# sdiehl/sonic

Hardware: AMD Instinct MI355X
Metric: prove() proofs/sec (higher is better)
Workload: dtype u32 limbs (Fq 12x32, Fr 8x32 Montgomery); 1 GPU; prove(): rndCircuit n=2^18, Q=2, SRS d=2^21 (d=8n >= 7n, Protocol.hs:54); n=262144, Q=2, d=2097152, process_group=none (plain single-process run), legs=headline only (the other legs: --full)

## Files before the change

### sonic_amd/csrc/field.hpp

```cpp
#pragma once
#include <stdint.h>
#include "constants.hpp"

#if defined(__HIP_DEVICE_COMPILE__) && !defined(SONIC_NO_ASM_MUL)
#define SONIC_FQ_LAZY 1
#else
#define SONIC_FQ_LAZY 0
#endif

#if defined(__HIPCC__)
#define HD __host__ __device__ __forceinline__
#define HD_NOINLINE __host__ __device__ __attribute__((noinline))
#else
#define HD inline __attribute__((always_inline))
#define HD_NOINLINE inline
#endif

namespace sonic {

struct FqParams {
  static constexpr int N = FQ_LIMBS;
  static constexpr uint32_t INV = FQ_INV;
  static constexpr bool LAZY = SONIC_FQ_LAZY != 0;
  static HD constexpr uint32_t p(int i) { constexpr uint32_t v[N] = FQ_P; return v[i]; }
// ... 177 lines not shown
    for (int j = 1; j < M; j++) {
      c += (u128)m * Pm[j] + t[j];
      t[j - 1] = (uint64_t)c;
      c >>= 64;
    }
    c += t[M];
    t[M - 1] = (uint64_t)c;
    t[M] = t[M + 1] + (uint64_t)(c >> 64);
  }
  Fp<P> r;
  for (int i = 0; i < M; i++) { r.l[2 * i] = (uint32_t)t[i]; r.l[2 * i + 1] = (uint32_t)(t[i] >> 32); }
  fp_reduce_once(r);
  return r;
}
#endif

}
#include "mont_asm.hpp"
namespace sonic {

template <class P>
HD Fp<P> fp_mul(const Fp<P>& a, const Fp<P>& b) {
#if defined(__HIP_DEVICE_COMPILE__) && !defined(SONIC_NO_ASM_MUL)
  if constexpr (P::N == FQ_LIMBS) return sonic_mont_mul_fq_call(a, b);
  else return sonic_mont_mul_fr_call(a, b);
#elif defined(__HIP_DEVICE_COMPILE__)
  return fp_mul_generic(a, b);
#else
  return fp_mul_host64(a, b);
#endif
}

template <class P>
HD Fp<P> fp_add(const Fp<P>& a, const Fp<P>& b) {
#if defined(__HIP_DEVICE_COMPILE__) && !defined(SONIC_NO_ASM_MUL)
  if constexpr (P::N == FQ_LIMBS) return sonic_fq_add_asm<P>(a, b);
  else return sonic_fr_add_asm<P>(a, b);
#else
  return fp_add_generic(a, b);
#endif
}
template <class P>
HD Fp<P> fp_sub(const Fp<P>& a, const Fp<P>& b) {
#if defined(__HIP_DEVICE_COMPILE__) && !defined(SONIC_NO_ASM_MUL)
  if constexpr (P::N == FQ_LIMBS) return sonic_fq_sub_asm<P>(a, b);
  else return sonic_fr_sub_asm<P>(a, b);
#else
  return fp_sub_generic(a, b);
#endif
}
template <class P>
HD Fp<P> fp_dbl(const Fp<P>& a) { return fp_add(a, a); }

template <class P>
HD Fp<P> fp_sqr(const Fp<P>& a) {
#if defined(__HIP_DEVICE_COMPILE__) && !defined(SONIC_NO_ASM_MUL)
  if constexpr (P::N == FQ_LIMBS) return sonic_mont_sqr_fq_call(a);
  else return fp_mul(a, a);
#else
  return fp_mul(a, a);
#endif
}

template <class P>
HD Fp<P> fp_to_mont(const Fp<P>& a) { return fp_mul(a, Fp<P>::r2()); }

template <class P>
HD Fp<P> fp_canonical(const Fp<P>& a) {
  Fp<P> r = a;
  if constexpr (P::LAZY) fp_reduce_once(r);
  return r;
}

template <class P>
HD bool Fp<P>::operator==(const Fp<P>& o) const {
  if constexpr (P::LAZY) return fp_sub(*this, o).is_zero();
  uint32_t t = 0;
  for (int i = 0; i < N; i++) t |= l[i] ^ o.l[i];
  return t == 0;
}

template <class P>
HD Fp<P> fp_from_mont(const Fp<P>& a) {
  Fp<P> o = Fp<P>::zero();
  o.l[0] = 1;
  return fp_canonical(fp_mul(a, o));
}

template <class P>
HD Fp<P> fp_pow_u64(const Fp<P>& a, uint64_t e) {
  Fp<P> acc = Fp<P>::one();
  bool started = false;
  for (int i = 63; i >= 0; i--) {
    if (started) acc = fp_sqr(acc);
    if ((e >> i) & 1) { acc = fp_mul(acc, a); started = true; }
  }
  return acc;
}

#if !defined(__HIP_DEVICE_COMPILE__)
template <class P>
inline Fp<P> fp_inv_euclid(const Fp<P>& a) {
  constexpr int N = P::N;
  if (a.is_zero()) return Fp<P>::zero();
  uint32_t u[N], v[N], x1[N], x2[N], pm[N];
  for (int i = 0; i < N; i++) { u[i] = a.l[i]; v[i] = pm[i] = P::p(i); x1[i] = 0; x2[i] = 0; }
// ... 84 lines not shown
```

### sonic_amd/csrc/g1.hpp

```cpp
#pragma once
#include "field.hpp"

namespace sonic {

struct G1Affine {
  Fq x, y;
  HD bool is_inf() const { return x.is_zero_strict() && y.is_zero_strict(); }
  static HD G1Affine inf() { G1Affine p; p.x = Fq::zero(); p.y = Fq::zero(); return p; }
};

#ifndef SONIC_SRS_POINT_BYTES
#define SONIC_SRS_POINT_BYTES 128
#endif
struct PointArray {
  const char* p;
  uint32_t stride;
  HD const G1Affine& operator[](size_t i) const { return *reinterpret_cast<const G1Affine*>(p + i * (size_t)stride); }
  HD PointArray operator+(long i) const { return PointArray{p + i * (long)stride, stride}; }
  static HD PointArray packed(const G1Affine* a) { return PointArray{reinterpret_cast<const char*>(a), (uint32_t)sizeof(G1Affine)}; }
};
struct PointArrayMut {
  char* p;
  uint32_t stride;
  HD G1Affine& operator[](size_t i) const { return *reinterpret_cast<G1Affine*>(p + i * (size_t)stride); }
  HD PointArrayMut operator+(long i) const { return PointArrayMut{p + i * (long)stride, stride}; }
  HD operator PointArray() const { return PointArray{p, stride}; }
};

struct G1XYZZ {
  Fq x, y, zz, zzz;
  HD bool is_inf() const { return zz.is_zero_strict(); }
  static HD G1XYZZ inf() {
    G1XYZZ p; p.x = Fq::zero(); p.y = Fq::zero(); p.zz = Fq::zero(); p.zzz = Fq::zero(); return p;
  }
  static HD G1XYZZ from_affine(const G1Affine& a) {
    G1XYZZ p;
    if (a.is_inf()) return inf();
    p.x = a.x; p.y = a.y; p.zz = Fq::one(); p.zzz = Fq::one();
    return p;
  }
};

HD G1Affine g1_neg(const G1Affine& p) { G1Affine r; r.x = p.x; r.y = fp_neg(p.y); return r; }
HD G1XYZZ g1_neg(const G1XYZZ& p) { G1XYZZ r = p; r.y = fp_neg(p.y); return r; }

HD G1XYZZ g1_dbl_affine(const G1Affine& p) {
  if (p.is_inf() || p.y.is_zero()) return G1XYZZ::inf();
  G1XYZZ r;
  Fq U = fp_dbl(p.y);
  Fq V = fp_sqr(U);
  Fq W = fp_mul(U, V);
  Fq S = fp_mul(p.x, V);
  Fq X2 = fp_sqr(p.x);
  Fq M = fp_add(fp_dbl(X2), X2);
  r.x = fp_sub(fp_sqr(M), fp_dbl(S));
  r.y = fp_sub(fp_mul(M, fp_sub(S, r.x)), fp_mul(W, p.y));
  r.zz = V;
  r.zzz = W;
  return r;
}

HD G1XYZZ g1_dbl(const G1XYZZ& p) {
  if (p.is_inf() || p.y.is_zero()) return G1XYZZ::inf();
  G1XYZZ r;
  Fq U = fp_dbl(p.y);
  Fq V = fp_sqr(U);
  Fq W = fp_mul(U, V);
  Fq S = fp_mul(p.x, V);
  Fq X2 = fp_sqr(p.x);
  Fq M = fp_add(fp_dbl(X2), X2);
  r.x = fp_sub(fp_sqr(M), fp_dbl(S));
  r.y = fp_sub(fp_mul(M, fp_sub(S, r.x)), fp_mul(W, p.y));
  r.zz = fp_mul(V, p.zz);
  r.zzz = fp_mul(W, p.zzz);
  return r;
}

HD G1XYZZ g1_add_mixed(const G1XYZZ& acc, const G1Affine& q) {
  if (q.is_inf()) return acc;
  if (acc.is_inf()) return G1XYZZ::from_affine(q);
  Fq U2 = fp_mul(q.x, acc.zz);
  Fq S2 = fp_mul(q.y, acc.zzz);
  Fq Pp = fp_sub(U2, acc.x);
  Fq R = fp_sub(S2, acc.y);
  if (Pp.is_zero()) {
    if (R.is_zero()) return g1_dbl_affine(q);
    return G1XYZZ::inf();
  }
  G1XYZZ r;
  Fq PP = fp_sqr(Pp);
  Fq PPP = fp_mul(Pp, PP);
  Fq Qv = fp_mul(acc.x, PP);
  r.x = fp_sub(fp_sub(fp_sqr(R), PPP), fp_dbl(Qv));
  r.y = fp_sub(fp_mul(R, fp_sub(Qv, r.x)), fp_mul(acc.y, PPP));
  r.zz = fp_mul(acc.zz, PP);
  r.zzz = fp_mul(acc.zzz, PPP);
  return r;
}

HD bool g1_in_subgroup_walk(const G1Affine& p) {
  constexpr uint32_t rl[8] = FR_P;
  G1XYZZ acc = G1XYZZ::from_affine(p);
#pragma unroll 1
  for (int b = 253; b >= 0; b--) {
    acc = g1_dbl(acc);
    uint32_t wd = 0;
#pragma unroll
    for (int k = 0; k < 8; k++) if (k == (b >> 5)) wd = rl[k];
    if ((wd >> (b & 31)) & 1u) acc = g1_add_mixed(acc, p);
  }
  return acc.is_inf();
}

HD Fq g1_endo_beta() {
  constexpr uint32_t b[12] = ENDO_BETA_MONT;
  Fq beta;
  for (int i = 0; i < 12; i++) beta.l[i] = b[i];
  return beta;
}

HD bool g1_in_subgroup(const G1Affine& p) {
  G1XYZZ acc = G1XYZZ::from_affine(p);
#pragma unroll 1
  for (int k = 0; k < 2; k++) {
    uint64_t w = k == 0 ? ENDO_Z2_HI << 1 : ENDO_Z2_LO;
    int left = k == 0 ? 63 : 64;
#pragma unroll 1
    while (left > 0) {
      const int run = w ? __builtin_clzll(w) + 1 : left;
#pragma unroll 1
      for (int i = 0; i < run; i++) acc = g1_dbl(acc);
      if (w) acc = g1_add_mixed(acc, p);
      w = run < 64 ? w << run : 0;
      left -= run;
    }
  }
  acc = g1_add_mixed(acc, g1_neg(p));
  if (acc.is_inf()) return false;
  return fp_mul(fp_mul(p.x, g1_endo_beta()), acc.zz) == acc.x && fp_mul(p.y, acc.zzz) == acc.y;
}

HD G1XYZZ g1_add_mixed_walk(G1XYZZ acc, const G1Affine& q, uint32_t negy = 0) {
#if SONIC_FQ_LAZY && !defined(SONIC_NO_FUSED_MADD)
  const uint32_t special = (acc.is_inf() || q.is_inf()) ? 1u : 0u;
  if (sonic_g1_madd_asm(acc, q.x, q.y, special, negy)) {
    G1Affine t = q;
    if (negy) t.y = fp_neg(t.y);
    acc = g1_add_mixed(acc, t);
  }
  return acc;
#else
  G1Affine t = q;
  if (negy) t.y = fp_neg(t.y);
  return g1_add_mixed(acc, t);
#endif
}

HD G1XYZZ g1_add_affine_walk(const G1Affine& first, const G1Affine& q, bool first_only) {
#if SONIC_FQ_LAZY && !defined(SONIC_NO_FUSED_MADD)
  G1XYZZ acc;
  acc.x = first.x; acc.y = first.y; acc.zz = Fq::one(); acc.zzz = Fq::one();
  const uint32_t special = (first_only || first.is_inf() || q.is_inf()) ? 1u : 0u;
  if (sonic_g1_aadd_asm(acc, q.x, q.y, special)) {
    acc = G1XYZZ::from_affine(first);
    if (!first_only) acc = g1_add_mixed(acc, q);
  }
  return acc;
#else
  G1XYZZ acc = G1XYZZ::from_affine(first);
  return first_only ? acc : g1_add_mixed(acc, q);
#endif
}

HD G1XYZZ g1_add(const G1XYZZ& p, const G1XYZZ& q) {
  if (q.is_inf()) return p;
  if (p.is_inf()) return q;
  Fq U1 = fp_mul(p.x, q.zz);
  Fq U2 = fp_mul(q.x, p.zz);
  Fq S1 = fp_mul(p.y, q.zzz);
  Fq S2 = fp_mul(q.y, p.zzz);
  Fq Pp = fp_sub(U2, U1);
  Fq R = fp_sub(S2, S1);
  if (Pp.is_zero()) {
    if (R.is_zero()) return g1_dbl(p);
    return G1XYZZ::inf();
  }
  G1XYZZ r;
  Fq PP = fp_sqr(Pp);
  Fq PPP = fp_mul(Pp, PP);
  Fq Qv = fp_mul(U1, PP);
  r.x = fp_sub(fp_sub(fp_sqr(R), PPP), fp_dbl(Qv));
  r.y = fp_sub(fp_mul(R, fp_sub(Qv, r.x)), fp_mul(S1, PPP));
  r.zz = fp_mul(fp_mul(p.zz, q.zz), PP);
  r.zzz = fp_mul(fp_mul(p.zzz, q.zzz), PPP);
  return r;
}

HD G1Affine g1_to_affine(const G1XYZZ& p) {
  if (p.is_inf()) return G1Affine::inf();
  Fq i = fp_inv(fp_mul(p.zz, p.zzz));
  G1Affine r;
  r.x = fp_mul(p.x, fp_mul(i, p.zzz));
  r.y = fp_mul(p.y, fp_mul(i, p.zz));
  return r;
}

HD G1XYZZ g1_mul_small(const G1XYZZ& p, uint32_t k) {
  G1XYZZ acc = G1XYZZ::inf();
  bool started = false;
  for (int i = 31; i >= 0; i--) {
    if (started) acc = g1_dbl(acc);
    if ((k >> i) & 1) { acc = g1_add(acc, p); started = true; }
  }
  return acc;
}

}
```

### sonic_amd/csrc/mont_asm.hpp

```cpp
#pragma once
#if defined(__HIP_DEVICE_COMPILE__)
namespace sonic {
extern "C" __device__ __attribute__((noinline, used)) void sonic_mont_mul_fq_holder() {
  asm volatile(
      ".pushsection .text.sonic_mont_mul_fq,\"ax\",@progbits\n\t"
      ".p2align 8\n\t"
      ".type sonic_mont_mul_fq,@function\n\t"
      "sonic_mont_mul_fq:\n\t"
      "s_mov_b32 s36, 0xffffaaab\n\t"
      "s_mov_b32 s37, 0xb9feffff\n\t"
      "s_mov_b32 s38, 0xb153ffff\n\t"
      "s_mov_b32 s39, 0x1eabfffe\n\t"
      "s_mov_b32 s40, 0xf6b0f624\n\t"
      "s_mov_b32 s41, 0x6730d2a0\n\t"
      "s_mov_b32 s42, 0xf38512bf\n\t"
      "s_mov_b32 s43, 0x64774b84\n\t"
      "s_mov_b32 s44, 0x434bacd7\n\t"
      "s_mov_b32 s45, 0x4b1ba7b6\n\t"
      "s_mov_b32 s46, 0x397fe69a\n\t"
      "s_mov_b32 s47, 0x1a0111ea\n\t"
      "s_mov_b32 s48, 0xfffcfffd\n\t"
      "v_mad_u64_u32 v[50:51], s[54:55], v0, v12, 0\n\t"
      "v_mad_u64_u32 v[52:53], s[54:55], v1, v12, 0\n\t"
      "v_mad_u64_u32 v[54:55], s[54:55], v2, v12, 0\n\t"
// ... 3727 lines not shown
      "v_mad_u64_u32 v[66:67], s[54:55], v107, v98, v[40:41]\n\t"
      "v_addc_co_u32_e64 v34, s[52:53], v60, v59, s[52:53]\n\t"
      "v_mad_u64_u32 v[56:57], s[54:55], v74, s39, v[30:31]\n\t"
      "v_addc_co_u32_e32 v46, vcc, v72, v71, vcc\n\t"
      "v_mad_u64_u32 v[68:69], s[54:55], v108, v98, v[42:43]\n\t"
      "v_addc_co_u32_e64 v36, s[52:53], v62, v61, s[52:53]\n\t"
      "v_mad_u64_u32 v[58:59], s[54:55], v74, s40, v[32:33]\n\t"
      "v_add_co_u32_e64 v24, s[50:51], v52, v51\n\t"
      "v_addc_co_u32_e32 v48, vcc, v48, v73, vcc\n\t"
      "v_mad_u64_u32 v[70:71], s[54:55], v109, v98, v[44:45]\n\t"
      "v_addc_co_u32_e64 v38, s[52:53], v64, v63, s[52:53]\n\t"
      "v_mad_u64_u32 v[60:61], s[54:55], v74, s41, v[34:35]\n\t"
      "v_addc_co_u32_e64 v26, s[50:51], v54, v53, s[50:51]\n\t"
      "v_mad_u64_u32 v[72:73], s[54:55], v110, v98, v[46:47]\n\t"
      "v_addc_co_u32_e64 v40, s[52:53], v66, v65, s[52:53]\n\t"
      "v_mad_u64_u32 v[62:63], s[54:55], v74, s42, v[36:37]\n\t"
      "v_addc_co_u32_e64 v28, s[50:51], v56, v55, s[50:51]\n\t"
      "v_addc_co_u32_e64 v42, s[52:53], v68, v67, s[52:53]\n\t"
      "v_mad_u64_u32 v[64:65], s[54:55], v74, s43, v[38:39]\n\t"
      "v_addc_co_u32_e64 v30, s[50:51], v58, v57, s[50:51]\n\t"
      "v_addc_co_u32_e64 v44, s[52:53], v70, v69, s[52:53]\n\t"
      "v_mad_u64_u32 v[66:67], s[54:55], v74, s44, v[40:41]\n\t"
      "v_addc_co_u32_e64 v32, s[50:51], v60, v59, s[50:51]\n\t"
      "v_addc_co_u32_e64 v46, s[52:53], v72, v71, s[52:53]\n\t"
      "v_mad_u64_u32 v[68:69], s[54:55], v74, s45, v[42:43]\n\t"
      "v_addc_co_u32_e64 v34, s[50:51], v62, v61, s[50:51]\n\t"
      "v_addc_co_u32_e64 v48, s[52:53], v48, v73, s[52:53]\n\t"
      "v_mad_u64_u32 v[70:71], s[54:55], v74, s46, v[44:45]\n\t"
      "v_addc_co_u32_e64 v36, s[50:51], v64, v63, s[50:51]\n\t"
      "v_mad_u64_u32 v[72:73], s[54:55], v74, s47, v[46:47]\n\t"
      "s_nop 0\n\t"
      "v_addc_co_u32_e64 v38, s[50:51], v66, v65, s[50:51]\n\t"
      "s_nop 0\n\t"
      "s_nop 0\n\t"
      "v_addc_co_u32_e64 v40, s[50:51], v68, v67, s[50:51]\n\t"
      "s_nop 0\n\t"
      "s_nop 0\n\t"
      "v_addc_co_u32_e64 v42, s[50:51], v70, v69, s[50:51]\n\t"
      "s_nop 0\n\t"
      "s_nop 0\n\t"
      "v_addc_co_u32_e64 v44, s[50:51], v72, v71, s[50:51]\n\t"
      "s_nop 0\n\t"
      "s_nop 0\n\t"
      "v_addc_co_u32_e64 v46, s[50:51], v48, v73, s[50:51]\n\t"
      "s_nop 0\n\t"
      "s_nop 0\n\t"
      "v_addc_co_u32_e64 v48, s[50:51], 0, 0, s[50:51]\n\t"
      "s_setpc_b64 s[30:31]\n\t"
      ".size sonic_mont_mul2_fq_core, .-sonic_mont_mul2_fq_core\n\t"
      ".popsection\n\t"
  );
}

template <class XYZZ, class F> __device__ __forceinline__ bool sonic_g1_madd_asm(XYZZ& acc, const F& qx, const F& qy, uint32_t special, uint32_t negy) {
  uint32_t exc;
  asm volatile(
      "s_mov_b32 s36, 0xffffaaab\n\t"
      "s_mov_b32 s37, 0xb9feffff\n\t"
      "s_mov_b32 s38, 0xb153ffff\n\t"
      "s_mov_b32 s39, 0x1eabfffe\n\t"
      "s_mov_b32 s40, 0xf6b0f624\n\t"
      "s_mov_b32 s41, 0x6730d2a0\n\t"
      "s_mov_b32 s42, 0xf38512bf\n\t"
      "s_mov_b32 s43, 0x64774b84\n\t"
      "s_mov_b32 s44, 0x434bacd7\n\t"
      "s_mov_b32 s45, 0x4b1ba7b6\n\t"
      "s_mov_b32 s46, 0x397fe69a\n\t"
      "s_mov_b32 s47, 0x1a0111ea\n\t"
      "s_mov_b32 s48, 0xfffcfffd\n\t"
      "v_mov_b32_e32 v25, 0\n\t"
      "v_mov_b32_e32 v27, 0\n\t"
      "v_mov_b32_e32 v29, 0\n\t"
      "v_mov_b32_e32 v31, 0\n\t"
      "v_mov_b32_e32 v33, 0\n\t"
      "v_mov_b32_e32 v35, 0\n\t"
      "v_mov_b32_e32 v37, 0\n\t"
      "v_mov_b32_e32 v39, 0\n\t"
      "v_mov_b32_e32 v41, 0\n\t"
      "v_mov_b32_e32 v43, 0\n\t"
      "v_mov_b32_e32 v45, 0\n\t"
      "v_mov_b32_e32 v47, 0\n\t"
      "v_mov_b32_e32 v49, 0\n\t"
      "v_mov_b32_e32 v48, 0\n\t"
      "s_mov_b64 s[60:61], exec\n\t"
      "v_cmp_ne_u32_e64 s[66:67], 0, %74\n\t"
      "v_sub_co_u32_e32 v50, vcc, 0xffff5556, %61\n\t"
      "v_mov_b32_e32 v63, 0x73fdffff\n\t"
      "v_mov_b32_e32 v64, 0x62a7ffff\n\t"
      "v_subb_co_u32_e32 v51, vcc, v63, %62, vcc\n\t"
      "v_mov_b32_e32 v65, 0x3d57fffd\n\t"
      "v_mov_b32_e32 v66, 0xed61ec48\n\t"
      "v_subb_co_u32_e32 v52, vcc, v64, %63, vcc\n\t"
      "v_mov_b32_e32 v67, 0xce61a541\n\t"
      "v_mov_b32_e32 v68, 0xe70a257e\n\t"
      "v_subb_co_u32_e32 v53, vcc, v65, %64, vcc\n\t"
      "v_mov_b32_e32 v69, 0xc8ee9709\n\t"
      "v_mov_b32_e32 v70, 0x869759ae\n\t"
      "v_subb_co_u32_e32 v54, vcc, v66, %65, vcc\n\t"
      "v_mov_b32_e32 v71, 0x96374f6c\n\t"
      "v_mov_b32_e32 v72, 0x72ffcd34\n\t"
      "v_subb_co_u32_e32 v55, vcc, v67, %66, vcc\n\t"
      "v_mov_b32_e32 v73, 0x340223d4\n\t"
      "v_mov_b32_e32 v12, %36\n\t"
      "v_subb_co_u32_e32 v56, vcc, v68, %67, vcc\n\t"
      "v_mov_b32_e32 v13, %37\n\t"
      "v_mov_b32_e32 v14, %38\n\t"
// ... 9185 lines not shown
```

### sonic_amd/csrc/msm.hip

```cpp
#include <string.h>
#include <stdexcept>
#include "internal.hpp"
#include "g1_quad.hpp"
#include "endo.hpp"

namespace sonic {

#ifndef SONIC_PART_LOW_BITS
#define SONIC_PART_LOW_BITS 8
#endif
constexpr int PART_LOW_BITS = SONIC_PART_LOW_BITS;
#ifndef SONIC_PART_TILE
#define SONIC_PART_TILE 1024
#endif
constexpr int PART_TILE = SONIC_PART_TILE;
constexpr uint32_t PASS1_GRID = 1024;
constexpr uint32_t PART_SORT_GRID = 2048;
#ifndef SONIC_PART_SORT_THREADS
#define SONIC_PART_SORT_THREADS 1024
#endif
constexpr int PART_SORT_THREADS = SONIC_PART_SORT_THREADS;
#ifndef SONIC_PART_SCATTER_THREADS
#define SONIC_PART_SCATTER_THREADS 512
#endif
constexpr int PART_SCATTER_THREADS = SONIC_PART_SCATTER_THREADS;
static_assert(PART_TILE % PART_SCATTER_THREADS == 0 && PART_SCATTER_THREADS >= 256, "a tile is a whole number of rounds of the workgroup");
static_assert(PART_LOW_BITS >= 8 && PART_LOW_BITS <= 10, "k_part_sort scans 256 x {1, 2, 4} counters");

static int g_window_override = 0;
int msm_window_override() { return g_window_override; }
void msm_set_window_override(int c) { g_window_override = c; }

#ifndef SONIC_HEAVY_THREADS
#define SONIC_HEAVY_THREADS 512
#endif
#ifndef SONIC_HEAVY_GRID
#define SONIC_HEAVY_GRID 256
#endif
static constexpr int HEAVY_THREADS = SONIC_HEAVY_THREADS;
static constexpr int HEAVY_GRID = SONIC_HEAVY_GRID;
static constexpr uint32_t HEAVY_MIN_STRETCH = 4 * HEAVY_THREADS;

struct HeavyMeta { uint32_t pad, n_heavy; uint32_t class_hist[256]; uint32_t class_cursor[256]; };
struct HeavyRec { uint32_t bucket, cnt, base, npart; };

static void plan_finish(MsmPlan& p, long n) {
  p.NB = 1 << (p.c - 1);
  p.K = p.NB < 8 ? p.NB : 8;
  p.nseg = p.NB / p.K;
  long mean = n * (long)(p.W / p.Wb) / p.NB;
  long t = 8 * mean;
  if (t < 256) t = 256;
  p.heavy_threshold = (uint32_t)t;
}

void msm_plan_set_segment(MsmPlan& p, int K) {
  if (K > p.NB) K = p.NB;
  if (K < 1) K = 1;
  while (K & (K - 1)) K &= K - 1;
  p.K = K;
  p.nseg = p.NB / K;
}

MsmPlan msm_plan(long n, bool fold) {
  MsmPlan p;
  p.fold = fold;
  int lg = 0;
  while ((1L << (lg + 1)) <= n) lg++;
  int c = lg - 4;
  if (c < 4) c = 4;
  if (c > 16) c = 16;
  if (g_window_override >= 4 && g_window_override <= 16) c = g_window_override;
  p.c = c;
  p.W = ((fold ? 255 : 256) + c - 1) / c;
// ... 220 lines not shown
    for (int k = 0; scans && k < per; k++) {
      const int t = threadIdx.x * per + k;
      if (t < P) { cur[t] = ex; delta[t] = base[row0 + (size_t)t * nblk] - ex; ex += hist[row0 + (size_t)t * nblk]; }
    }
    if (threadIdx.x == 0) total_sh = tot;
    __syncthreads();
    for (int k = 0; k < PART_TILE / T; k++) {
      const long i = (long)blk * PART_TILE + k * T + threadIdx.x;
      DigitStream ds;
      ds.init(scal, i, i < n, mont, fold);
      for (int w = 0; w < W; w++) {
        uint32_t sign;
        const uint32_t d = ds.next(keystride ? c : msm_even_width(W, w, batch.bits), sign);
        const uint32_t key = (uint32_t)w * keystride + d - 1;
        const uint32_t pr = key >> PART_LOW_BITS;
        const uint32_t pos = lds_take(cur, d != 0, pr);
        if (d) {
          const uint32_t lo = key & ((1u << PART_LOW_BITS) - 1), hi = (uint32_t)i | (keystride ? 0u : (uint32_t)w << 26) | (sign << 31);
          recs[pos] = make_uint2(lo, hi);
          pid[pos] = (uint16_t)pr;
        }
      }
    }
    __syncthreads();
    const uint32_t total = total_sh;
    for (uint32_t i = threadIdx.x; i < total; i += T) part[delta[pid[i]] + i] = recs[i];
    __syncthreads();
  }
}

__global__ __launch_bounds__(PART_SORT_THREADS) void k_part_sort(const MsmBatchDev batch, const uint2* __restrict__ part,
                                                   const uint32_t* __restrict__ base, const uint32_t* __restrict__ total, size_t hn, int P,
                                                   uint32_t jobstride, uint32_t* __restrict__ off, uint32_t* __restrict__ entries, uint32_t* __restrict__ class_hist,
                                                   uint32_t stage_cap) {
  extern __shared__ uint32_t stage[];
  __shared__ uint32_t cnt[1 << PART_LOW_BITS];
  __shared__ uint32_t sc4[256];
  __shared__ uint32_t chist[256];
  const uint32_t M = (uint32_t)batch.k * jobstride;
  const uint32_t nparts = (uint32_t)batch.k * (uint32_t)P;
  constexpr uint32_t T = PART_SORT_THREADS;
  if (threadIdx.x < 256) chist[threadIdx.x] = 0;
  for (uint32_t pi = blockIdx.x; pi < nparts; pi += gridDim.x) {
  const int job = pi / P, t = pi % P;
  const uint32_t nblk = batch.tile0[job + 1] - batch.tile0[job];
  const size_t idx = (size_t)P * batch.tile0[job] + (size_t)t * nblk, idx_next = idx + nblk;
  const uint32_t beg = idx < hn ? base[idx] : *total;
  const uint32_t end = idx_next < hn ? base[idx_next] : *total;
  const bool last_block = pi == nparts - 1;
  for (int t = threadIdx.x; t < (1 << PART_LOW_BITS); t += T) cnt[t] = 0;
  __syncthreads();
  const uint32_t span = end - beg, trips = (span + T - 1) / T;
  constexpr int B = 8;
  for (uint32_t k0 = 0; k0 < trips; k0 += B) {
    uint32_t lo[B];
#pragma unroll
    for (int j = 0; j < B; j++) { const uint32_t e = beg + (k0 + j) * T + threadIdx.x; lo[j] = e < end ? part[e].x : 0xffffffffu; }
#pragma unroll
    for (int j = 0; j < B; j++) if (k0 + j < trips) lds_take(cnt, lo[j] != 0xffffffffu, lo[j] & ((1u << PART_LOW_BITS) - 1));
  }
  __syncthreads();
  constexpr int CPT = (1 << PART_LOW_BITS) / 256;
  const bool scans = threadIdx.x < 256;
  uint32_t v[CPT], ssum = 0;
  for (int k = 0; k < CPT; k++) { v[k] = scans ? cnt[threadIdx.x * CPT + k] : 0u; ssum += v[k]; }
  uint32_t ex = block_exclusive_scan_256(ssum, sc4, nullptr);
  for (int k = 0; scans && k < CPT; k++) {
    const uint32_t local = (uint32_t)t * (1u << PART_LOW_BITS) + threadIdx.x * CPT + k;
    cnt[threadIdx.x * CPT + k] = ex;
    if (local < jobstride) { off[(uint32_t)job * jobstride + local] = beg + ex; atomicAdd(&chist[size_class(v[k])], 1u); }
    ex += v[k];
  }
  if (last_block && threadIdx.x == 0) off[M] = *total;
  __syncthreads();
  for (uint32_t k0 = 0; k0 < trips; k0 += B) {
    uint32_t lo[B], pay[B];
#pragma unroll
    for (int j = 0; j < B; j++) {
      const uint32_t e = beg + (k0 + j) * T + threadIdx.x;
      const bool live = e < end;
      const uint2 rec = live ? part[e] : make_uint2(0xffffffffu, 0u);
      lo[j] = rec.x;
      pay[j] = rec.y;
    }
#pragma unroll
    for (int j = 0; j < B; j++) {
      if (k0 + j >= trips) continue;
      const bool live = lo[j] != 0xffffffffu;
      const uint32_t pos = lds_take(cnt, live, lo[j] & ((1u << PART_LOW_BITS) - 1));
      if (live) { if (span <= stage_cap) stage[pos] = pay[j]; else entries[beg + pos] = pay[j]; }
    }
  }
  __syncthreads();
  if (span <= stage_cap) {
    for (uint32_t i = threadIdx.x; i < span; i += T) entries[beg + i] = stage[i];
    __syncthreads();
  }
  }
  const uint32_t c = threadIdx.x < 256 ? chist[threadIdx.x] : 0u;
  if (c) atomicAdd(&class_hist[threadIdx.x], c);
}

__device__ __forceinline__ uint32_t block_exclusive_scan_256(uint32_t v, uint32_t* sh, uint32_t* total) {
  const int t = threadIdx.x;
  const bool in = t < 256;
  if (in) sh[t] = v;
  __syncthreads();
  for (int o = 1; o < 256; o <<= 1) {
    uint32_t x = in && t >= o ? sh[t - o] : 0;
    __syncthreads();
    if (in) sh[t] += x;
    __syncthreads();
  }
  uint32_t incl = in ? sh[t] : 0u;
  if (total) *total = sh[255];
  __syncthreads();
  return incl - v;
}
__global__ __launch_bounds__(256) void k_scan_tile_sums(const uint32_t* in, size_t m, uint32_t* tile_sums) {
  __shared__ uint32_t sh[256];
  size_t base = (size_t)blockIdx.x * 2048 + threadIdx.x * 8;
  uint32_t s = 0;
  for (int k = 0; k < 8; k++) if (base + k < m) s += in[base + k];
  uint32_t tot;
  block_exclusive_scan_256(s, sh, &tot);
  if (threadIdx.x == 0) tile_sums[blockIdx.x] = tot;
}
__global__ __launch_bounds__(256) void k_scan_top(uint32_t* tile_sums, int ntiles, uint32_t* total_out) {
  __shared__ uint32_t sh[256];
  __shared__ uint32_t carry_sh;
  if (threadIdx.x == 0) carry_sh = 0;
  __syncthreads();
  for (int base = 0; base < ntiles; base += 256) {
    int idx = base + threadIdx.x;
    uint32_t v = idx < ntiles ? tile_sums[idx] : 0, tot;
    uint32_t ex = block_exclusive_scan_256(v, sh, &tot);
    uint32_t carry = carry_sh;
    if (idx < ntiles) tile_sums[idx] = ex + carry;
    __syncthreads();
    if (threadIdx.x == 0) carry_sh = carry + tot;
    __syncthreads();
  }
  if (threadIdx.x == 0) *total_out = carry_sh;
}
// ... 237 lines not shown
    }
    reinterpret_cast<Fq*>(&sh[q])[cr] = acc;
    __syncthreads();
    for (int sp = 8; sp >= 1; sp >>= 1) {
      if (q < sp && (uint32_t)(q + sp) < r.npart) {
        Fq* pa = reinterpret_cast<Fq*>(&sh[q]) + cr;
        *pa = g1q_add(*pa, reinterpret_cast<const Fq*>(&sh[q + sp])[cr], cr);
      }
      __syncthreads();
    }
    if (threadIdx.x < 4) reinterpret_cast<Fq*>(&buckets[r.bucket])[threadIdx.x] = reinterpret_cast<const Fq*>(&sh[0])[threadIdx.x];
    __syncthreads();
  }
}

#ifndef SONIC_SEGMENTS_LDS_TOT
#define SONIC_SEGMENTS_LDS_TOT 1
#endif
struct LdsPoint {
  uint32_t* base;
  __device__ __forceinline__ void store(const G1XYZZ& p) const {
    const uint32_t* w = reinterpret_cast<const uint32_t*>(&p);
#pragma unroll
    for (int k = 0; k < 48; k++) base[k * 256] = w[k];
  }
  __device__ __forceinline__ G1XYZZ load() const {
    G1XYZZ p;
    uint32_t* w = reinterpret_cast<uint32_t*>(&p);
#pragma unroll
    for (int k = 0; k < 48; k++) w[k] = base[k * 256];
    return p;
  }
  __device__ __forceinline__ Fq coord(int i) const {
    Fq f;
#pragma unroll
    for (int k = 0; k < 12; k++) f.l[k] = base[(12 * i + k) * 256];
    return f;
  }
  __device__ __forceinline__ void set_coord(int i, const Fq& f) const {
#pragma unroll
    for (int k = 0; k < 12; k++) base[(12 * i + k) * 256] = f.l[k];
  }
  __device__ __forceinline__ void add(const G1XYZZ& q) const {
    if (q.is_inf()) return;
    const Fq pzz = coord(2);
    if (pzz.is_zero_strict()) { store(q); return; }
    const Fq U1 = fp_mul(coord(0), q.zz);
    const Fq U2 = fp_mul(q.x, pzz);
    const Fq S1 = fp_mul(coord(1), q.zzz);
    const Fq S2 = fp_mul(q.y, coord(3));
    const Fq Pp = fp_sub(U2, U1);
    const Fq R = fp_sub(S2, S1);
    if (Pp.is_zero()) {
      store(R.is_zero() ? g1_dbl(load()) : G1XYZZ::inf());
      return;
    }
    const Fq PP = fp_sqr(Pp);
    const Fq PPP = fp_mul(Pp, PP);
    const Fq Qv = fp_mul(U1, PP);
    const Fq x = fp_sub(fp_sub(fp_sqr(R), PPP), fp_dbl(Qv));
    set_coord(0, x);
    set_coord(1, fp_sub(fp_mul(R, fp_sub(Qv, x)), fp_mul(S1, PPP)));
    set_coord(2, fp_mul(fp_mul(coord(2), q.zz), PP));
    set_coord(3, fp_mul(fp_mul(coord(3), q.zzz), PPP));
  }
};
template <bool RUNS>
__global__ __launch_bounds__(256, SONIC_SEGMENTS_LDS_TOT ? 2 : 1) void k_bucket_segments(const G1XYZZ* __restrict__ buckets, int W, int NB, int K, int nseg,
                                                        G1XYZZ* __restrict__ segres, G1XYZZ* __restrict__ runs) {
#if SONIC_SEGMENTS_LDS_TOT
  __shared__ uint32_t tot_sh[48 * 256];
  const LdsPoint tl{tot_sh + threadIdx.x};
#endif
  int t = blockIdx.x * blockDim.x + threadIdx.x;
  if (t >= W * nseg) return;
  const int w = t / nseg, sg = t % nseg;
  const G1XYZZ* B = buckets + (size_t)w * NB + (size_t)sg * K;
  G1XYZZ run = G1XYZZ::inf();
#if SONIC_SEGMENTS_LDS_TOT
  tl.store(G1XYZZ::inf());
  for (int j = K - 1; j >= 0; j--) {
    run = g1_add(run, B[j]);
    tl.add(run);
  }
#else
  G1XYZZ tot = G1XYZZ::inf();
  for (int j = K - 1; j >= 0; j--) {
    run = g1_add(run, B[j]);
    tot = g1_add(tot, run);
  }
#endif
  if (RUNS) {
    runs[t] = run;
#if SONIC_SEGMENTS_LDS_TOT
    segres[t] = tl.load();
#else
    segres[t] = tot;
#endif
    return;
  }
  const int k0 = sg * K;
  G1XYZZ acc = G1XYZZ::inf();
  bool have_multiple = false;
  if (nseg % 64 == 0) {
    const uint32_t hi = __builtin_amdgcn_readfirstlane((uint32_t)sg >> 6), lo = (uint32_t)sg & 63u;
    for (int i = 31 - __clz((int)(hi | 1u)); i >= 0; i--) {
      acc = g1_dbl(acc);
      if ((hi >> i) & 1u) acc = g1_add(acc, run);
    }
    for (int i = 5; i >= 0; i--) {
      acc = g1_dbl(acc);
      if ((lo >> i) & 1u) acc = g1_add(acc, run);
    }
    for (int s = K; s > 1; s >>= 1) acc = g1_dbl(acc);
    have_multiple = true;
  } else if (k0) {
    acc = g1_mul_small(run, (uint32_t)k0);
    have_multiple = true;
  }
#if SONIC_SEGMENTS_LDS_TOT
  G1XYZZ tot = tl.load();
#endif
  if (have_multiple) tot = g1_add(tot, acc);
  segres[t] = tot;
}

__global__ __launch_bounds__(256, 2) void k_window_sum(const G1XYZZ* __restrict__ segres, int W, int c, int nseg, int runs_L, int K, const MsmBatchDev batch) {
  __shared__ G1XYZZ sh[256];
  const int w = blockIdx.x % W;
  MsmSlot* slot = batch.slot[blockIdx.x / W];
  segres += (size_t)(blockIdx.x - w) * nseg;
  G1XYZZ acc = G1XYZZ::inf();
  for (int s = threadIdx.x; s < nseg; s += 256) acc = g1_add(acc, segres[(size_t)w * nseg + s]);
  sh[threadIdx.x] = acc;
  __syncthreads();
  for (int s = 128; s >= 1; s >>= 1) {
    if ((int)threadIdx.x < s) sh[threadIdx.x] = g1_add(sh[threadIdx.x], sh[threadIdx.x + s]);
    __syncthreads();
  }
  if (threadIdx.x == 0) {
    G1XYZZ r = sh[0];
    r.x = fp_canonical(r.x); r.y = fp_canonical(r.y); r.zz = fp_canonical(r.zz); r.zzz = fp_canonical(r.zzz);
    if (runs_L > 0) { slot->win[runs_L] = r; slot->W = runs_L; slot->c = 1; slot->pad0 = K; slot->pad1 = 3; return; }
    slot->win[w] = r;
    if (w == 0) { slot->W = W; slot->c = c; slot->pad0 = 0; slot->pad1 = 0; }
  }
}

__global__ __launch_bounds__(256, 2) void k_group_sum(const G1XYZZ* __restrict__ in, long n_in, int group, G1XYZZ* __restrict__ out) {
  __shared__ G1XYZZ sh[256];
  const long base = (long)blockIdx.x * group;
  G1XYZZ acc = G1XYZZ::inf();
  for (long s = threadIdx.x; s < group && base + s < n_in; s += 256) acc = g1_add(acc, in[base + s]);
  sh[threadIdx.x] = acc;
  __syncthreads();
  for (int s = 128; s >= 1; s >>= 1) {
    if ((int)threadIdx.x < s) sh[threadIdx.x] = g1_add(sh[threadIdx.x], sh[threadIdx.x + s]);
    __syncthreads();
  }
  if (threadIdx.x == 0) out[blockIdx.x] = sh[0];
}

constexpr int TREE_BLOCK_LOG = 10;
constexpr int TREE_MID_LOG = 14;
#ifndef SONIC_TREE_LATENCY_MAX
#define SONIC_TREE_LATENCY_MAX (1L << 17)
#endif
constexpr long TREE_LATENCY_MAX_BUCKETS = SONIC_TREE_LATENCY_MAX;
constexpr int TREE_LATENCY_BLOCK_LOG = 7, TREE_LATENCY_MID_LOG = 12;

__device__ __forceinline__ void tree_item(G1XYZZ* __restrict__ Z, size_t s0, int m, uint32_t it) {
  const uint32_t pair = it / (uint32_t)m, comp = it % (uint32_t)m;
  const size_t s = s0 + ((size_t)pair << m);
  const size_t pos = comp == 0 ? 0 : (size_t)1 << (comp - 1);
  const size_t h = (size_t)1 << (m - 1);
  Z[s + pos] = g1_add(Z[s + pos], Z[s + h + pos]);
// ... 310 lines not shown
```

Measured before the change: 31.75 proofs/s.

## Add fused two-product Montgomery multiply for curve Y, and register-ranked partition sort

Adds a fused asm routine that computes a*b + c*d with a single Montgomery reduction and uses it for the Y coordinate in the doubling and addition formulas, replacing two separate multiplies and a subtraction. The bucket-segment scalar ladder keeps the old path through a template flag, likely to limit register pressure there. Separately, the partition sort now keeps up to 12 records per thread in registers together with their LDS ranks, so the second pass can skip re-reading global memory and re-running the atomics. The LDS point add also now doubles q instead of reloading the point on the equal-points case. The extra asm call clobbers many VGPRs and the register arrays in the sort may hurt occupancy.

```diff
diff --git a/sonic_amd/csrc/field.hpp b/sonic_amd/csrc/field.hpp
--- a/sonic_amd/csrc/field.hpp
+++ b/sonic_amd/csrc/field.hpp
@@ -253,6 +253,30 @@
 template <class P>
 HD Fp<P> fp_dbl(const Fp<P>& a) { return fp_add(a, a); }
 
+#if SONIC_FQ_LAZY && !defined(SONIC_NO_TWO_PRODUCT)
+#define SONIC_FQ_TWO_PRODUCT 1
+#else
+#define SONIC_FQ_TWO_PRODUCT 0
+#endif
+template <class P>
+HD Fp<P> fp_mul2(const Fp<P>& a, const Fp<P>& b, const Fp<P>& c, const Fp<P>& d) {
+#if SONIC_FQ_TWO_PRODUCT
+  if constexpr (P::N == FQ_LIMBS) return sonic_mont_mul2_fq_call(a, b, c, d);
+  else return fp_add(fp_mul(a, b), fp_mul(c, d));
+#else
+  return fp_add(fp_mul(a, b), fp_mul(c, d));
+#endif
+}
+template <class P>
+HD Fp<P> fp_mul2_diff(const Fp<P>& a, const Fp<P>& b, const Fp<P>& c, const Fp<P>& d) {
+#if SONIC_FQ_TWO_PRODUCT
+  if constexpr (P::N == FQ_LIMBS) return sonic_mont_mul2_fq_call(a, b, fp_neg(c), d);
+  else return fp_sub(fp_mul(a, b), fp_mul(c, d));
+#else
+  return fp_sub(fp_mul(a, b), fp_mul(c, d));
+#endif
+}
+
 template <class P>
 HD Fp<P> fp_sqr(const Fp<P>& a) {
 #if defined(__HIP_DEVICE_COMPILE__) && !defined(SONIC_NO_ASM_MUL)
diff --git a/sonic_amd/csrc/g1.hpp b/sonic_amd/csrc/g1.hpp
--- a/sonic_amd/csrc/g1.hpp
+++ b/sonic_amd/csrc/g1.hpp
@@ -54,12 +54,13 @@
   Fq X2 = fp_sqr(p.x);
   Fq M = fp_add(fp_dbl(X2), X2);
   r.x = fp_sub(fp_sqr(M), fp_dbl(S));
-  r.y = fp_sub(fp_mul(M, fp_sub(S, r.x)), fp_mul(W, p.y));
+  r.y = fp_mul2_diff(M, fp_sub(S, r.x), p.y, W);
   r.zz = V;
   r.zzz = W;
   return r;
 }
 
+template <bool TWO_PRODUCT = true>
 HD G1XYZZ g1_dbl(const G1XYZZ& p) {
   if (p.is_inf() || p.y.is_zero()) return G1XYZZ::inf();
   G1XYZZ r;
@@ -70,7 +71,8 @@
   Fq X2 = fp_sqr(p.x);
   Fq M = fp_add(fp_dbl(X2), X2);
   r.x = fp_sub(fp_sqr(M), fp_dbl(S));
-  r.y = fp_sub(fp_mul(M, fp_sub(S, r.x)), fp_mul(W, p.y));
+  if constexpr (TWO_PRODUCT) r.y = fp_mul2_diff(M, fp_sub(S, r.x), p.y, W);
+  else r.y = fp_sub(fp_mul(M, fp_sub(S, r.x)), fp_mul(W, p.y));
   r.zz = fp_mul(V, p.zz);
   r.zzz = fp_mul(W, p.zzz);
   return r;
@@ -92,7 +94,7 @@
   Fq PPP = fp_mul(Pp, PP);
   Fq Qv = fp_mul(acc.x, PP);
   r.x = fp_sub(fp_sub(fp_sqr(R), PPP), fp_dbl(Qv));
-  r.y = fp_sub(fp_mul(R, fp_sub(Qv, r.x)), fp_mul(acc.y, PPP));
+  r.y = fp_mul2_diff(R, fp_sub(Qv, r.x), acc.y, PPP);
   r.zz = fp_mul(acc.zz, PP);
   r.zzz = fp_mul(acc.zzz, PPP);
   return r;
@@ -172,6 +174,7 @@
 #endif
 }
 
+template <bool TWO_PRODUCT = true>
 HD G1XYZZ g1_add(const G1XYZZ& p, const G1XYZZ& q) {
   if (q.is_inf()) return p;
   if (p.is_inf()) return q;
@@ -182,7 +185,7 @@
   Fq Pp = fp_sub(U2, U1);
   Fq R = fp_sub(S2, S1);
   if (Pp.is_zero()) {
-    if (R.is_zero()) return g1_dbl(p);
+    if (R.is_zero()) return g1_dbl<TWO_PRODUCT>(p);
     return G1XYZZ::inf();
   }
   G1XYZZ r;
@@ -190,9 +193,10 @@
   Fq PPP = fp_mul(Pp, PP);
   Fq Qv = fp_mul(U1, PP);
   r.x = fp_sub(fp_sub(fp_sqr(R), PPP), fp_dbl(Qv));
-  r.y = fp_sub(fp_mul(R, fp_sub(Qv, r.x)), fp_mul(S1, PPP));
   r.zz = fp_mul(fp_mul(p.zz, q.zz), PP);
   r.zzz = fp_mul(fp_mul(p.zzz, q.zzz), PPP);
+  if constexpr (TWO_PRODUCT) r.y = fp_mul2_diff(R, fp_sub(Qv, r.x), S1, PPP);
+  else r.y = fp_sub(fp_mul(R, fp_sub(Qv, r.x)), fp_mul(S1, PPP));
   return r;
 }
 
@@ -205,12 +209,13 @@
   return r;
 }
 
+template <bool TWO_PRODUCT = true>
 HD G1XYZZ g1_mul_small(const G1XYZZ& p, uint32_t k) {
   G1XYZZ acc = G1XYZZ::inf();
   bool started = false;
   for (int i = 31; i >= 0; i--) {
-    if (started) acc = g1_dbl(acc);
-    if ((k >> i) & 1) { acc = g1_add(acc, p); started = true; }
+    if (started) acc = g1_dbl<TWO_PRODUCT>(acc);
+    if ((k >> i) & 1) { acc = g1_add<TWO_PRODUCT>(acc, p); started = true; }
   }
   return acc;
 }
diff --git a/sonic_amd/csrc/mont_asm.hpp b/sonic_amd/csrc/mont_asm.hpp
--- a/sonic_amd/csrc/mont_asm.hpp
+++ b/sonic_amd/csrc/mont_asm.hpp
@@ -3803,6 +3803,106 @@
   );
 }
 
+__device__ __forceinline__ Fp<FqParams> sonic_mont_mul2_fq_call(const Fp<FqParams>& a, const Fp<FqParams>& b, const Fp<FqParams>& c, const Fp<FqParams>& d) {
+  Fp<FqParams> r;
+  asm volatile(
+      "s_mov_b32 s36, 0xffffaaab\n\t"
+      "s_mov_b32 s37, 0xb9feffff\n\t"
+      "s_mov_b32 s38, 0xb153ffff\n\t"
+      "s_mov_b32 s39, 0x1eabfffe\n\t"
+      "s_mov_b32 s40, 0xf6b0f624\n\t"
+      "s_mov_b32 s41, 0x6730d2a0\n\t"
+      "s_mov_b32 s42, 0xf38512bf\n\t"
+      "s_mov_b32 s43, 0x64774b84\n\t"
+      "s_mov_b32 s44, 0x434bacd7\n\t"
+      "s_mov_b32 s45, 0x4b1ba7b6\n\t"
+      "s_mov_b32 s46, 0x397fe69a\n\t"
+      "s_mov_b32 s47, 0x1a0111ea\n\t"
+      "s_mov_b32 s48, 0xfffcfffd\n\t"
+      "v_mov_b32_e32 v25, 0\n\t"
+      "v_mov_b32_e32 v27, 0\n\t"
+      "v_mov_b32_e32 v29, 0\n\t"
+      "v_mov_b32_e32 v31, 0\n\t"
+      "v_mov_b32_e32 v33, 0\n\t"
+      "v_mov_b32_e32 v35, 0\n\t"
+      "v_mov_b32_e32 v37, 0\n\t"
+      "v_mov_b32_e32 v39, 0\n\t"
+      "v_mov_b32_e32 v41, 0\n\t"
+      "v_mov_b32_e32 v43, 0\n\t"
+      "v_mov_b32_e32 v45, 0\n\t"
+      "v_mov_b32_e32 v47, 0\n\t"
+      "v_mov_b32_e32 v49, 0\n\t"
+      "v_mov_b32_e32 v48, 0\n\t"
+      "v_mov_b32_e32 v0, %12\n\t"
+      "v_mov_b32_e32 v1, %13\n\t"
+      "v_mov_b32_e32 v2, %14\n\t"
+      "v_mov_b32_e32 v3, %15\n\t"
+      "v_mov_b32_e32 v4, %16\n\t"
+      "v_mov_b32_e32 v5, %17\n\t"
+      "v_mov_b32_e32 v6, %18\n\t"
+      "v_mov_b32_e32 v7, %19\n\t"
+      "v_mov_b32_e32 v8, %20\n\t"
+      "v_mov_b32_e32 v9, %21\n\t"
+      "v_mov_b32_e32 v10, %22\n\t"
+      "v_mov_b32_e32 v11, %23\n\t"
+      "v_mov_b32_e32 v12, %24\n\t"
+      "v_mov_b32_e32 v13, %25\n\t"
+      "v_mov_b32_e32 v14, %26\n\t"
+      "v_mov_b32_e32 v15, %27\n\t"
+      "v_mov_b32_e32 v16, %28\n\t"
+      "v_mov_b32_e32 v17, %29\n\t"
+      "v_mov_b32_e32 v18, %30\n\t"
+      "v_mov_b32_e32 v19, %31\n\t"
+      "v_mov_b32_e32 v20, %32\n\t"
+      "v_mov_b32_e32 v21, %33\n\t"
+      "v_mov_b32_e32 v22, %34\n\t"
+      "v_mov_b32_e32 v23, %35\n\t"
+      "v_mov_b32_e32 v99, %36\n\t"
+      "v_mov_b32_e32 v100, %37\n\t"
+      "v_mov_b32_e32 v101, %38\n\t"
+      "v_mov_b32_e32 v102, %39\n\t"
+      "v_mov_b32_e32 v103, %40\n\t"
+      "v_mov_b32_e32 v104, %41\n\t"
+      "v_mov_b32_e32 v105, %42\n\t"
+      "v_mov_b32_e32 v106, %43\n\t"
+      "v_mov_b32_e32 v107, %44\n\t"
+      "v_mov_b32_e32 v108, %45\n\t"
+      "v_mov_b32_e32 v109, %46\n\t"
+      "v_mov_b32_e32 v110, %47\n\t"
+      "v_mov_b32_e32 v87, %48\n\t"
+      "v_mov_b32_e32 v88, %49\n\t"
+      "v_mov_b32_e32 v89, %50\n\t"
+      "v_mov_b32_e32 v90, %51\n\t"
+      "v_mov_b32_e32 v91, %52\n\t"
+      "v_mov_b32_e32 v92, %53\n\t"
+      "v_mov_b32_e32 v93, %54\n\t"
+      "v_mov_b32_e32 v94, %55\n\t"
+      "v_mov_b32_e32 v95, %56\n\t"
+      "v_mov_b32_e32 v96, %57\n\t"
+      "v_mov_b32_e32 v97, %58\n\t"
+      "v_mov_b32_e32 v98, %59\n\t"
+      "s_getpc_b64 s[56:57]\n\t"
+      "s_add_u32 s56, s56, sonic_mont_mul2_fq_core@rel32@lo+4\n\t"
+      "s_addc_u32 s57, s57, sonic_mont_mul2_fq_core@rel32@hi+12\n\t"
+      "s_swappc_b64 s[30:31], s[56:57]\n\t"
+      "v_mov_b32_e32 %0, v24\n\t"
+      "v_mov_b32_e32 %1, v26\n\t"
+      "v_mov_b32_e32 %2, v28\n\t"
+      "v_mov_b32_e32 %3, v30\n\t"
+      "v_mov_b32_e32 %4, v32\n\t"
+      "v_mov_b32_e32 %5, v34\n\t"
+      "v_mov_b32_e32 %6, v36\n\t"
+      "v_mov_b32_e32 %7, v38\n\t"
+      "v_mov_b32_e32 %8, v40\n\t"
+      "v_mov_b32_e32 %9, v42\n\t"
+      "v_mov_b32_e32 %10, v44\n\t"
+      "v_mov_b32_e32 %11, v46"
+      : "=v"(r.l[0]), "=v"(r.l[1]), "=v"(r.l[2]), "=v"(r.l[3]), "=v"(r.l[4]), "=v"(r.l[5]), "=v"(r.l[6]), "=v"(r.l[7]), "=v"(r.l[8]), "=v"(r.l[9]), "=v"(r.l[10]), "=v"(r.l[11])
+      : "v"(a.l[0]), "v"(a.l[1]), "v"(a.l[2]), "v"(a.l[3]), "v"(a.l[4]), "v"(a.l[5]), "v"(a.l[6]), "v"(a.l[7]), "v"(a.l[8]), "v"(a.l[9]), "v"(a.l[10]), "v"(a.l[11]), "v"(b.l[0]), "v"(b.l[1]), "v"(b.l[2]), "v"(b.l[3]), "v"(b.l[4]), "v"(b.l[5]), "v"(b.l[6]), "v"(b.l[7]), "v"(b.l[8]), "v"(b.l[9]), "v"(b.l[10]), "v"(b.l[11]), "v"(c.l[0]), "v"(c.l[1]), "v"(c.l[2]), "v"(c.l[3]), "v"(c.l[4]), "v"(c.l[5]), "v"(c.l[6]), "v"(c.l[7]), "v"(c.l[8]), "v"(c.l[9]), "v"(c.l[10]), "v"(c.l[11]), "v"(d.l[0]), "v"(d.l[1]), "v"(d.l[2]), "v"(d.l[3]), "v"(d.l[4]), "v"(d.l[5]), "v"(d.l[6]), "v"(d.l[7]), "v"(d.l[8]), "v"(d.l[9]), "v"(d.l[10]), "v"(d.l[11])
+      : "v0", "v1", "v2", "v3", "v4", "v5", "v6", "v7", "v8", "v9", "v10", "v11", "v12", "v13", "v14", "v15", "v16", "v17", "v18", "v19", "v20", "v21", "v22", "v23", "v24", "v25", "v26", "v27", "v28", "v29", "v30", "v31", "v32", "v33", "v34", "v35", "v36", "v37", "v38", "v39", "v40", "v41", "v42", "v43", "v44", "v45", "v46", "v47", "v48", "v49", "v50", "v51", "v52", "v53", "v54", "v55", "v56", "v57", "v58", "v59", "v60", "v61", "v62", "v63", "v64", "v65", "v66", "v67", "v68", "v69", "v70", "v71", "v72", "v73", "v74", "v87", "v88", "v89", "v90", "v91", "v92", "v93", "v94", "v95", "v96", "v97", "v98", "v99", "v100", "v101", "v102", "v103", "v104", "v105", "v106", "v107", "v108", "v109", "v110", "s30", "s31", "s36", "s37", "s38", "s39", "s40", "s41", "s42", "s43", "s44", "s45", "s46", "s47", "s48", "s49", "s50", "s51", "s52", "s53", "s54", "s55", "s56", "s57", "vcc", "scc");
+  return r;
+}
+
 template <class XYZZ, class F> __device__ __forceinline__ bool sonic_g1_madd_asm(XYZZ& acc, const F& qx, const F& qy, uint32_t special, uint32_t negy) {
   uint32_t exc;
   asm volatile(
diff --git a/sonic_amd/csrc/msm.hip b/sonic_amd/csrc/msm.hip
--- a/sonic_amd/csrc/msm.hip
+++ b/sonic_amd/csrc/msm.hip
@@ -20,6 +20,9 @@
 #define SONIC_PART_SORT_THREADS 1024
 #endif
 constexpr int PART_SORT_THREADS = SONIC_PART_SORT_THREADS;
+#ifndef SORT_RANK_TRIPS
+#define SORT_RANK_TRIPS 12
+#endif
 #ifndef SONIC_PART_SCATTER_THREADS
 #define SONIC_PART_SCATTER_THREADS 512
 #endif
@@ -346,12 +349,30 @@
   __syncthreads();
   const uint32_t span = end - beg, trips = (span + T - 1) / T;
   constexpr int B = 8;
+  constexpr int RT = SORT_RANK_TRIPS > 0 ? SORT_RANK_TRIPS : 1;
+  const bool ranked = trips <= (uint32_t)SORT_RANK_TRIPS;
+  uint32_t rlo[RT], rpay[RT], rrank[RT];
+  if (ranked) {
+#pragma unroll
+    for (int j = 0; j < RT; j++) {
+      const uint32_t e = beg + (uint32_t)j * T + threadIdx.x;
+      const uint2 rec = e < end ? part[e] : make_uint2(0xffffffffu, 0u);
+      rlo[j] = rec.x;
+      rpay[j] = rec.y;
+    }
+#pragma unroll
+    for (int j = 0; j < RT; j++) {
+      rrank[j] = 0;
+      if ((uint32_t)j < trips) rrank[j] = lds_take(cnt, rlo[j] != 0xffffffffu, rlo[j] & ((1u << PART_LOW_BITS) - 1));
+    }
+  } else {
   for (uint32_t k0 = 0; k0 < trips; k0 += B) {
     uint32_t lo[B];
 #pragma unroll
     for (int j = 0; j < B; j++) { const uint32_t e = beg + (k0 + j) * T + threadIdx.x; lo[j] = e < end ? part[e].x : 0xffffffffu; }
 #pragma unroll
     for (int j = 0; j < B; j++) if (k0 + j < trips) lds_take(cnt, lo[j] != 0xffffffffu, lo[j] & ((1u << PART_LOW_BITS) - 1));
+  }
   }
   __syncthreads();
   constexpr int CPT = (1 << PART_LOW_BITS) / 256;
@@ -367,6 +388,14 @@
   }
   if (last_block && threadIdx.x == 0) off[M] = *total;
   __syncthreads();
+  if (ranked) {
+#pragma unroll
+    for (int j = 0; j < RT; j++) {
+      if (rlo[j] == 0xffffffffu) continue;
+      const uint32_t pos = cnt[rlo[j] & ((1u << PART_LOW_BITS) - 1)] + rrank[j];
+      if (span <= stage_cap) stage[pos] = rpay[j]; else entries[beg + pos] = rpay[j];
+    }
+  } else {
   for (uint32_t k0 = 0; k0 < trips; k0 += B) {
     uint32_t lo[B], pay[B];
 #pragma unroll
@@ -384,6 +413,7 @@
       const uint32_t pos = lds_take(cnt, live, lo[j] & ((1u << PART_LOW_BITS) - 1));
       if (live) { if (span <= stage_cap) stage[pos] = pay[j]; else entries[beg + pos] = pay[j]; }
     }
+  }
   }
   __syncthreads();
   if (span <= stage_cap) {
@@ -727,7 +757,7 @@
     const Fq Pp = fp_sub(U2, U1);
     const Fq R = fp_sub(S2, S1);
     if (Pp.is_zero()) {
-      store(R.is_zero() ? g1_dbl(load()) : G1XYZZ::inf());
+      store(R.is_zero() ? g1_dbl(q) : G1XYZZ::inf());
       return;
     }
     const Fq PP = fp_sqr(Pp);
@@ -735,9 +765,9 @@
     const Fq Qv = fp_mul(U1, PP);
     const Fq x = fp_sub(fp_sub(fp_sqr(R), PPP), fp_dbl(Qv));
     set_coord(0, x);
-    set_coord(1, fp_sub(fp_mul(R, fp_sub(Qv, x)), fp_mul(S1, PPP)));
     set_coord(2, fp_mul(fp_mul(coord(2), q.zz), PP));
     set_coord(3, fp_mul(fp_mul(coord(3), q.zzz), PPP));
+    set_coord(1, fp_mul2_diff(R, fp_sub(Qv, x), S1, PPP));
   }
 };
 template <bool RUNS>
@@ -780,23 +810,23 @@
   if (nseg % 64 == 0) {
     const uint32_t hi = __builtin_amdgcn_readfirstlane((uint32_t)sg >> 6), lo = (uint32_t)sg & 63u;
     for (int i = 31 - __clz((int)(hi | 1u)); i >= 0; i--) {
-      acc = g1_dbl(acc);
-      if ((hi >> i) & 1u) acc = g1_add(acc, run);
+      acc = g1_dbl<false>(acc);
+      if ((hi >> i) & 1u) acc = g1_add<false>(acc, run);
     }
     for (int i = 5; i >= 0; i--) {
-      acc = g1_dbl(acc);
-      if ((lo >> i) & 1u) acc = g1_add(acc, run);
-    }
-    for (int s = K; s > 1; s >>= 1) acc = g1_dbl(acc);
+      acc = g1_dbl<false>(acc);
+      if ((lo >> i) & 1u) acc = g1_add<false>(acc, run);
+    }
+    for (int s = K; s > 1; s >>= 1) acc = g1_dbl<false>(acc);
     have_multiple = true;
   } else if (k0) {
-    acc = g1_mul_small(run, (uint32_t)k0);
+    acc = g1_mul_small<false>(run, (uint32_t)k0);
     have_multiple = true;
   }
 #if SONIC_SEGMENTS_LDS_TOT
   G1XYZZ tot = tl.load();
 #endif
-  if (have_multiple) tot = g1_add(tot, acc);
+  if (have_multiple) tot = g1_add<false>(tot, acc);
   segres[t] = tot;
 }
 
```

Result: slower. 31.27 proofs/s (-1.5%).
